# Infinidat/slimfastq

Measured on AMD Instinct MI355X. Metric: MB/s FASTQ compressed, higher is better.
Workload: dtype u8/u32 integer; 1 GPU; synthetic 10M x 150 bp Illumina reads per GPU, full qlts+gens+recs, frozen tables (one chain per lane), -l 3; level=3, block_reads=1024, prior_step=-1, blocks_per_gpu=9766, tables=frozen, chains_per_gpu=253906, raw_bytes_per_gpu=3702038404, parallelism=1 GPU

## Files before the change

### slimfastq_amd/csrc/chains.hip

```cpp
#include "kernels.h"
#include "dev_chain.h"
#include "dev_walk.h"
typedef u32 __attribute__((aligned(1))) u32_any;

#define LAST_QLT 63u
#define QROW_BYTES 256u
#define B2_INIT 0x03030303u

#define QDEC_ROW 72u
__device__ __forceinline__ void qdec_store(u16* row, u32 s, u32 cum) {
    if (s) row[8 + s - 1] = (u16)cum;
    if ((s & 7u) == 0) row[s >> 3] = (u16)cum;
    if (s == 63) row[8 + 63] = 0;
}
__global__ __launch_bounds__(256) void k_qlt_frozen_rows(const u32* __restrict__ rows66, u32 q_rows, u32* __restrict__ qrows, u16* __restrict__ qdec) {
    const u32 lane = threadIdx.x & 63;
    const u32 ctx = blockIdx.x * 4 + (threadIdx.x >> 6);
    if (ctx >= q_rows) return;
    const u32* r = rows66 + (size_t)ctx * 66;
    const u32 slot = r[lane], iend = r[65];
    if (iend == 0) {
        qrows[(size_t)ctx * 64 + lane] = (lane << 10) | (1024u << 16);
        if (qdec) qdec_store(qdec + (size_t)ctx * QDEC_ROW, lane, lane << 10);
        return;
    }
    const u32 sym = slot >> 16, fslot = lane < iend ? (slot & 0xffffu) : 0u;
    const u32 f = (u32)__builtin_amdgcn_ds_permute((int)((lane < iend ? sym : lane) * 4), (int)fslot);
    const u32 x = f + 1;
    u32 S = x;
#pragma unroll
    for (int d = 32; d > 0; d >>= 1) S += (u32)__shfl_xor((int)S, d, 64);
    u32 g = (x << 16) / S;
    g = g ? g : 1u;
    u32 sum = g, best = (g << 6) | (63u - lane);
#pragma unroll
    for (int d = 32; d > 0; d >>= 1) {
        sum += (u32)__shfl_xor((int)sum, d, 64);
        const u32 o = (u32)__shfl_xor((int)best, d, 64); best = o > best ? o : best;
    }
    if (lane == 63u - (best & 63u)) g += 65536u - sum;
    u32 incl = g;
#pragma unroll
    for (int d = 1; d < 64; d <<= 1) { const u32 o = (u32)__shfl_up((int)incl, d, 64); if (lane >= (u32)d) incl += o; }
    qrows[(size_t)ctx * 64 + lane] = (incl - g) | (g << 16);
    if (qdec) qdec_store(qdec + (size_t)ctx * QDEC_ROW, lane, incl - g);
}
void launch_qlt_frozen_rows(const u32* rows66, u32 q_rows, u32* qrows, u16* qdec, hipStream_t st) {
    hipLaunchKernelGGL(k_qlt_frozen_rows, dim3((q_rows + 3) / 4), dim3(256), 0, st, rows66, q_rows, qrows, qdec);
}

#define QH_SYMS 48u
#define QH_ROW_U16 50u
#define QH_MAP_BYTES(q_rows) ((q_rows) / 32u * 8u)
#define QH_EMPTY 0xFFFFFFFFu
__global__ __launch_bounds__(256) void k_hot_totals(const u32* __restrict__ hist, const u32* __restrict__ rows66, u32 q_rows, u32* __restrict__ ctot) {
    const u32 lane = threadIdx.x & 63;
    const u32 ctx = blockIdx.x * 4 + (threadIdx.x >> 6);
    if (ctx >= q_rows) return;
    u32 c = hist[(size_t)ctx * 64 + lane];
#pragma unroll
    for (int d = 32; d > 0; d >>= 1) c += (u32)__shfl_xor((int)c, d, 64);
    const u32 iend = rows66[(size_t)ctx * 66 + 65];
    if (lane == 0) ctot[ctx] = (iend != 0 && iend <= QH_SYMS) ? c : 0u;
}
__global__ __launch_bounds__(1024) void k_hot_select(const u32* __restrict__ ctot, u32 q_rows, u32 want, uint2* __restrict__ map, u32* __restrict__ info) {
    __shared__ u32 red[16];
    __shared__ u32 wbits[2048];
    const u32 t = threadIdx.x, lane = t & 63, wave = t >> 6;
    const u32 nwords = q_rows / 32u;
    u32 c[64];
    u32 mx = 0;
#pragma unroll
    for (u32 k = 0; k < 64; k++) {
        const u32 ctx = k * 1024u + t;
        c[k] = ctx < q_rows ? ctot[ctx] : 0u;
        mx = c[k] > mx ? c[k] : mx;
    }
    auto block_sum = [&](u32 v) {
#pragma unroll
        for (int d = 32; d > 0; d >>= 1) v += (u32)__shfl_xor((int)v, d, 64);
        __syncthreads();
        if (lane == 0) red[wave] = v;
        __syncthreads();
        u32 s2 = 0;
        for (u32 w = 0; w < 16; w++) s2 += red[w];
        return s2;
    };
    auto block_max = [&](u32 v) {
#pragma unroll
        for (int d = 32; d > 0; d >>= 1) { const u32 o = (u32)__shfl_xor((int)v, d, 64); v = o > v ? o : v; }
        __syncthreads();
        if (lane == 0) red[wave] = v;
        __syncthreads();
        u32 s2 = 0;
        for (u32 w = 0; w < 16; w++) s2 = red[w] > s2 ? red[w] : s2;
        return s2;
    };
    u32 lo = 1, hi = block_max(mx) + 1u;
    while (lo < hi) {
        const u32 mid = lo + (hi - lo) / 2u;
        u32 n = 0;
#pragma unroll
        for (u32 k = 0; k < 64; k++) n += c[k] >= mid;
        if (block_sum(n) <= want) hi = mid; else lo = mid + 1u;
    }
    const u32 T = lo;
#pragma unroll
    for (u32 k = 0; k < 64; k++) {
        const u64 m = __ballot(c[k] >= T);
        if (lane == 0) { wbits[k * 32u + wave * 2u] = (u32)m; wbits[k * 32u + wave * 2u + 1u] = (u32)(m >> 32); }
    }
    __syncthreads();
    const u32 b0 = 2u * t < nwords ? wbits[2u * t] : 0u, b1 = 2u * t + 1u < nwords ? wbits[2u * t + 1u] : 0u;
    const u32 mine = (u32)__popc(b0) + (u32)__popc(b1);
    u32 inc = mine;
#pragma unroll
    for (int d = 1; d < 64; d <<= 1) { const u32 o = (u32)__shfl_up((int)inc, d, 64); if (lane >= (u32)d) inc += o; }
    __syncthreads();
    if (lane == 63) red[wave] = inc;
    __syncthreads();
    u32 before = 0, all = 0;
    for (u32 w = 0; w < 16; w++) { const u32 v = red[w]; before += w < wave ? v : 0u; all += v; }
    const u32 rank = before + inc - mine;
    if (t == 0) info[0] = all;
    if (2u * t < nwords) map[2u * t] = make_uint2(b0, rank);
    if (2u * t + 1u < nwords) map[2u * t + 1u] = make_uint2(b1, rank + (u32)__popc(b0));
}
__global__ __launch_bounds__(256) void k_hot_image(const uint2* __restrict__ map, const u32* __restrict__ qrows, u32 q_rows, u16* __restrict__ rows) {
    const u32 lane = threadIdx.x & 63;
    const u32 ctx = blockIdx.x * 4 + (threadIdx.x >> 6);
    if (ctx >= q_rows) return;
    const uint2 mr = map[ctx >> 5];
    const u32 bit = 1u << (ctx & 31u);
    if (!(mr.x & bit)) return;
    const u32 slot = mr.y + (u32)__popc(mr.x & (bit - 1u));
    if (lane < QH_ROW_U16) rows[(size_t)slot * QH_ROW_U16 + lane] = lane <= QH_SYMS ? (u16)FZ_CUM(qrows[(size_t)ctx * 64 + lane]) : (u16)0;
}
void launch_hot_rows(const u32* hist, const u32* rows66, const u32* qrows, u32 q_rows, u32 want, u32* ctot, u8* img, u32* info, hipStream_t st) {
    hipLaunchKernelGGL(k_hot_totals, dim3((q_rows + 3) / 4), dim3(256), 0, st, hist, rows66, q_rows, ctot);
    hipLaunchKernelGGL(k_hot_select, dim3(1), dim3(1024), 0, st, (const u32*)ctot, q_rows, want, reinterpret_cast<uint2*>(img), info);
    hipLaunchKernelGGL(k_hot_image, dim3((q_rows + 3) / 4), dim3(256), 0, st, reinterpret_cast<const uint2*>(img), qrows, q_rows,
                       reinterpret_cast<u16*>(img + QH_MAP_BYTES(q_rows)));
}

#define QHD_ROW_U16 8u
#define QHD_MAX_ROWS 6000u
__global__ __launch_bounds__(256) void k_hot_totals_prior(const u32* __restrict__ rows66, u32 q_rows, u32* __restrict__ ctot) {
    const u32 ctx = blockIdx.x * 256 + threadIdx.x;
    if (ctx >= q_rows) return;
    const u32 iend = rows66[(size_t)ctx * 66 + 65];
    ctot[ctx] = iend != 0 ? rows66[(size_t)ctx * 66 + 64] + 1u : 0u;
}
__global__ __launch_bounds__(256) void k_hot_image_dec(const uint2* __restrict__ map, const u16* __restrict__ qdec, u32 q_rows, u16* __restrict__ rows) {
    const u32 ctx = blockIdx.x * 256 + threadIdx.x;
    if (ctx >= q_rows) return;
// ... 551 lines not shown
        __syncthreads();
    }
}
__device__ __forceinline__ u32 gen_row_of(uint4 n, u32 step) {
    u64 f0 = 3 + (u64)step * n.x, f1 = 3 + (u64)step * n.y, f2 = 3 + (u64)step * n.z, f3 = 3 + (u64)step * n.w;
    while ((f0 | f1 | f2 | f3) > 255) {
        f0 = (f0 >> 1) | (f0 & 1); f1 = (f1 >> 1) | (f1 & 1); f2 = (f2 >> 1) | (f2 & 1); f3 = (f3 >> 1) | (f3 & 1);
    }
    return (u32)f0 | (u32)f1 << 8 | (u32)f2 << 16 | (u32)f3 << 24;
}
__global__ __launch_bounds__(1024) void k_gen_bin_count(const u16* __restrict__ bins, u32* __restrict__ fill, u32 cap, u32 g_bits, u32* __restrict__ cnt,
                                                        u32* __restrict__ rows_out, u32 step) {
    extern __shared__ u32 lds[];
    const u32 sb = gb_slice_bits(g_bits), nctx = 1u << sb, b = blockIdx.x, tid = threadIdx.x;
    u32 n = fill[b]; if (n > cap) n = cap;
    const u16* bin = bins + (size_t)b * cap;
    uint4* slice = reinterpret_cast<uint4*>(cnt + ((size_t)b << (sb + 2)));
    if (!n && !rows_out) return;
    for (u32 at = 0; ; at += 65535u) {
        for (u32 i = tid; i < 2u * nctx; i += 1024u) lds[i] = 0;
        __syncthreads();
        const u32 m = n - at < 65535u ? n - at : 65535u;
        for (u32 i = tid; i < m; i += 1024u) {
            const u32 k = bin[at + i];
            atomicAdd(&lds[k >> 1], 1u << ((k & 1u) * 16u));
        }
        __syncthreads();
        const bool last_chunk = at + m >= n;
        for (u32 i = tid; i < nctx; i += 1024u) {
            const u32 w0 = lds[2 * i], w1 = lds[2 * i + 1];
            if (!(w0 | w1) && !(rows_out && last_chunk)) continue;
            uint4 c = slice[i];
            c.x += w0 & 0xffffu; c.y += w0 >> 16; c.z += w1 & 0xffffu; c.w += w1 >> 16;
            if (w0 | w1) slice[i] = c;
            if (rows_out && last_chunk) rows_out[((size_t)b << sb) + i] = gen_row_of(c, step);
        }
        if (last_chunk) break;
        __syncthreads();
    }
    if (tid == 0) fill[b] = 0;
}
GenBins gen_bins_plan(u32 g_bits, u64 max_keys) {
    GenBins gb; gb.bins = nullptr; gb.fill = nullptr;
    gb.g_bits = g_bits;
    gb.batch = max_keys < GEN_BIN_BATCH ? (max_keys ? max_keys : 1) : GEN_BIN_BATCH;
    const u32 nb = 1u << (g_bits - gb_slice_bits(g_bits));
    gb.cap = (u32)((2ull * ((gb.batch + nb - 1) / nb) + 4096ull + 63ull) & ~63ull);
    gb.bins_bytes = (u64)gb.cap * 2ull * nb; gb.fill_bytes = 4ull * nb;
    return gb;
}
void launch_gen_count_binned(const ChainArgs& a, u32 b0, u32 b1, u64 nrec_range, u32 max_line, const GenBins& gb, u32* cnt, u32* rows_out, u32 step,
                             hipStream_t st, u32 sub) {
    const u32 g_bits = gb.g_bits, sb = gb_slice_bits(g_bits), nb = 1u << (g_bits - sb), cap = gb.cap;
    const u32 dyn2 = (2u << sb) * 4u;
    static u32 allowed = 0;
    if (dyn2 > 65536u && dyn2 > allowed) { (void)hipFuncSetAttribute(reinterpret_cast<const void*>(&k_gen_bin_count), hipFuncAttributeMaxDynamicSharedMemorySize, (int)dyn2); allowed = dyn2; }
    if (nrec_range) {
        u32 stride = gen_count_stride(nrec_range);
        if (sub == 1) { stride *= GEN_PRE; sub = 0; }
        u32 seg_len = 0;
        if (max_line >= 64u) {
            const u64 nsel = (nrec_range + stride - 1) / stride;
            for (u32 sl = 32u; sl < max_line && sl <= 512u; sl *= 2u)
                if (nsel * ((max_line + sl - 1) / sl) <= 524288ull) { seg_len = sl; break; }
        }
        if (!seg_len && max_line > 1024u) seg_len = 512u;
        const u32 segs = seg_len ? (max_line + seg_len - 1) / seg_len : 1u;
        const u64 lanes = ((nrec_range + stride - 1) / stride) * segs;
        const u64 per_lane = seg_len ? seg_len : (max_line ? max_line : 1u);
        u64 lanes_per_batch = gb.batch / per_lane; if (!lanes_per_batch) lanes_per_batch = 1;
        lanes_per_batch = (lanes_per_batch + GB_T - 1) / GB_T * GB_T;
        const u32 dyn1 = (GB_TILE + 2u * nb) * 4u;
        for (u64 id0 = 0; id0 < lanes; id0 += lanes_per_batch) {
            const u64 id1 = id0 + lanes_per_batch < lanes ? id0 + lanes_per_batch : lanes;
            const bool last = id1 >= lanes;
            hipLaunchKernelGGL(k_gen_bin, dim3((u32)((id1 - id0 + GB_T - 1) / GB_T)), dim3(GB_T), dyn1, st, a, b0, b1, stride, seg_len, segs, sub, id0, id1, g_bits, gb.bins, gb.fill, cap, cnt);
            hipLaunchKernelGGL(k_gen_bin_count, dim3(nb), dim3(1024), dyn2, st, (const u16*)gb.bins, gb.fill, cap, g_bits, cnt, last ? rows_out : nullptr, step);
        }
    } else if (rows_out) hipLaunchKernelGGL(k_gen_bin_count, dim3(nb), dim3(1024), dyn2, st, (const u16*)gb.bins, gb.fill, cap, g_bits, cnt, rows_out, step);
}

__global__ __launch_bounds__(256) void k_gen_rows(const u32* __restrict__ cnt, u32* __restrict__ rows, u64 nctx, u32 step) {
    const u64 c = (u64)blockIdx.x * 256 + threadIdx.x;
    if (c >= nctx) return;
    const uint4 n = *reinterpret_cast<const uint4*>(cnt + c * 4);
    u64 f0 = 3 + (u64)step * n.x, f1 = 3 + (u64)step * n.y, f2 = 3 + (u64)step * n.z, f3 = 3 + (u64)step * n.w;
    while ((f0 | f1 | f2 | f3) > 255) {
        f0 = (f0 >> 1) | (f0 & 1); f1 = (f1 >> 1) | (f1 & 1); f2 = (f2 >> 1) | (f2 & 1); f3 = (f3 >> 1) | (f3 & 1);
    }
    rows[c] = (u32)f0 | (u32)f1 << 8 | (u32)f2 << 16 | (u32)f3 << 24;
}
void launch_gen_rows(const u32* cnt, u32* rows, u64 nctx, u32 step, hipStream_t st) {
    hipLaunchKernelGGL(k_gen_rows, dim3((u32)((nctx + 255) / 256)), dim3(256), 0, st, cnt, rows, nctx, step);
}

__device__ __forceinline__ const u32* gen_rows_of(const ChainArgs& a, u32 b) {
    if (!a.g_ngen) return nullptr;
    u32 g = 0;
    while (g + 1 < a.g_ngen && b >= a.g_bound[g + 1]) g++;
    return a.g_rows[g];
}

#define GEN_RING 8
template <int THREADS, bool FLAT>
__global__ __launch_bounds__(THREADS) void k_gen_encode_c(ChainArgs a, u32 c0, u32 c1 ) {
    __shared__ u32 rcp[FLAT ? 1 : 1024];
    __shared__ u8 lut[256];
    __shared__ u32 ring[LaneEncB<THREADS, GEN_RING>::LDS_DWORDS];
    if constexpr (!FLAT) for (u32 i = threadIdx.x; i < 1024; i += THREADS) rcp[i] = i ? rc_recip(i) : 0u;
    for (u32 i = threadIdx.x; i < 256; i += THREADS) lut[i] = (u8)(gen_code_of(i) | (is_lower_base(i) ? 0x20u : 0u));
    __syncthreads();
    const u32 c = c0 + blockIdx.x * THREADS + threadIdx.x;
    const bool live = c < c1;
    ChainPos cp; cp.b = 0; cp.r0 = 0; cp.nrec = 0; cp.sub_lo = cp.sub_len = 0; cp.seg = 0; cp.nseg = 1;
    if (live) { cp = chain_pos(a, c); chain_seg_encode(a, cp); }
    const BlockDesc* d = &a.m.blocks[cp.b];
    LaneEncB<THREADS, GEN_RING> rc; u32 cap = 0;
    u8* outp = live ? chain_region(a, cp, SFQ_S_GEN, 3, 4, cap) : nullptr;
    rc.init(ring, threadIdx.x, outp, cap);
    const u32* rows = (!FLAT && live) ? gen_rows_of(a, cp.b) : nullptr;
    u32 illegal = 0;
    if (a.flat_quads && (FLAT || !__any(rows != nullptr))) {
        illegal = walk_bases_q(a, cp.r0, cp.nrec, live ? d->solid : 0u, lut,
            [&](u32 sym, u32 k) { const u32 bits = 2u * k; rc.encode_bits_if(k ? ~0u : 0u, sym & ((1u << bits) - 1u), 1u, bits); rc.drain(); },
            a.exc_flag, cp.sub_lo, cp.sub_len);
    } else if (FLAT || !__any(rows != nullptr)) {
        const u32 r12 = rc_recip(12u);
        illegal = walk_bases_b(a, cp.r0, cp.nrec, live ? d->solid : 0u, 0u, lut, [&](u32, u32) {},
            [&](u32, u32 code, u32 vm) { rc.encode_if(vm, 3u * code, 3u, 12u, r12); },
            [&]() { rc.drain(); }, a.exc_flag, cp.sub_lo, cp.sub_len);
    } else if constexpr (!FLAT) {
        const u32* rp = rows ? rows : a.g_init;
        const u32 mask = (live && rows) ? (1u << d->gen_bits) - 1u : 0u;
        u32 rv[16];
        illegal = walk_bases_b(a, cp.r0, cp.nrec, live ? d->solid : 0u, mask, lut,
            [&](u32 j, u32 ctx) { rv[j] = rp[ctx]; },
            [&](u32 j, u32 code, u32 vm) {
                const u32 v = rv[j];
                const u32 f0 = v & 0xff, f1 = (v >> 8) & 0xff, f2 = (v >> 16) & 0xff, f3 = v >> 24;
                const u32 tot = (f0 + f1) + (f2 + f3);
                const u32 below = v & ((1u << (8 * code)) - 1u);
                const u32 cum = (below & 0xff) + ((below >> 8) & 0xff) + (below >> 16);
                rc.encode_if(vm, cum, (v >> (8 * code)) & 0xff, tot, rcp[tot]);
            },
            [&]() { rc.drain(); }, a.exc_flag, cp.sub_lo, cp.sub_len);
    }
    if (live) {
        a.csz[c] = rc.finish();
        if (rc.err & 2) atomicMax(&a.m.blocks[cp.b].status, (u32)(-SFQ_E_OVERFLOW));
        else if (rc.err) atomicMax(&a.m.blocks[cp.b].status, (u32)(-SFQ_E_CORRUPT));
        if (illegal) atomicMax(&a.m.blocks[cp.b].status, (u32)(-SFQ_E_GENCHAR));
    }
}
__device__ __forceinline__ uint4 gp_below(u32 n) {
    const u64 lo = n >= 8u ? ~0ull : (1ull << (8u * n)) - 1ull;
    const u64 hi = n >= 16u ? ~0ull : n <= 8u ? 0ull : (1ull << (8u * (n - 8u))) - 1ull;
    return make_uint4((u32)lo, (u32)(lo >> 32), (u32)hi, (u32)(hi >> 32));
}
__device__ __forceinline__ uint4 gp_load16(const u8* buf, u64 nbytes, long long at) {
    if (at >= 0 && (u64)at + 16u <= nbytes) return load16(buf, nbytes, (u64)at);
    u32 w[4] = {0, 0, 0, 0};
    for (u32 i = 0; i < 16; i++) { const long long p = at + (long long)i; if (p >= 0 && (u64)p < nbytes) w[i >> 2] |= (u32)buf[p] << ((i & 3) * 8); }
    return make_uint4(w[0], w[1], w[2], w[3]);
}
__device__ __forceinline__ u32 gp_codes(u32 w, u32 valid, u32& odd, u32& ill) {
    const u32 s1 = w >> 1;
    u32 cd = (s1 ^ (w >> 2)) & 0x03030303u;
    const u32 want = __builtin_amdgcn_perm(0u, 0x47544341u, s1 & 0x03030303u);
    odd = 0; ill = 0;
    if ((want ^ w) & valid) {
        cd = 0;
#pragma unroll
        for (u32 i = 0; i < 4; i++) {
            const u32 ch = (w >> (8u * i)) & 0xffu, g = gen_code_of(ch);
            cd |= (g & 3u) << (8u * i);
            if ((valid >> (8u * i)) & 0xffu) {
                if (g > 3u || is_lower_base(ch)) odd |= 0x80u << (8u * i);
                if (g & 0x10u) ill = 1;
            }
        }
    }
    return cd & valid & 0x03030303u;
}
__device__ __forceinline__ u32 gp_fold(u32 cd) { return cd | (cd >> 6); }
__device__ __forceinline__ u32 gp_nib(u32 t) { return ((t >> 7) * 0x01020408u) >> 24; }
__device__ __forceinline__ u32 gp_bits16(u32 o0, u32 o1, u32 o2, u32 o3) { return gp_nib(o0) | gp_nib(o1) << 4 | gp_nib(o2) << 8 | gp_nib(o3) << 12; }
__global__ __launch_bounds__(256) void k_gen_pack_raw(ChainArgs a, u32 c0, u32 c1) {
    const u32 lane = threadIdx.x & 63u;
    const u32 c = c0 + blockIdx.x * 4u + (threadIdx.x >> 6);
    if (c >= c1) return;
    ChainPos cp = chain_pos(a, c); chain_seg_encode(a, cp);
    const u32 solid = a.m.blocks[cp.b].solid;
    u32 cap = 0;
    u32* out = reinterpret_cast<u32*>(chain_region(a, cp, SFQ_S_GEN, 3, 4, cap));
    const u8* buf = a.st_off ? a.st_buf : a.m.fq;
    const u64 nbytes = a.st_off ? a.st_bytes : a.nbytes;
    u32 done = 0;
    u32 carry = 0;
    u32 illegal = 0;
    for (u32 k0 = 0; k0 < cp.nrec; k0 += 64u) {
        const u32 k = k0 + lane;
        u64 b0 = 0, b1 = 0;
        if (k < cp.nrec) {
            const u64 r = cp.r0 + k;
            if (a.st_off) { b0 = a.st_off[r]; b1 = b0 + a.st_len[r]; }
            else { b0 = a.m.line_off[4 * r + 1] + solid; b1 = a.m.line_off[4 * r + 2] - 1; }
            if (cp.sub_len) {
                if (b1 < b0) b1 = b0;
                const u64 lo = b0 + cp.sub_lo;
                b0 = lo < b1 ? lo : b1;
                b1 = b0 + cp.sub_len < b1 ? b0 + cp.sub_len : b1;
            }
            if (b1 < b0) b1 = b0;
        }
        const u32 len = (u32)(b1 - b0);
        u32 inc = len;
#pragma unroll
        for (int d = 1; d < 64; d <<= 1) { const u32 o = (u32)__shfl_up((int)inc, d, 64); if (lane >= (u32)d) inc += o; }
        const u32 st = inc - len;
        const u32 tot = (u32)__shfl((int)inc, 63, 64);
        const u32 end = done + tot;
        const bool last_chunk = k0 + 64u >= cp.nrec;
        const u32 t0 = done >> 4, t1 = (end + 15u) >> 4;
        for (u32 tb = t0; tb < t1; tb += 64u) {
            const u32 t = tb + lane;
            const u32 d0 = 16u * t;
            const u32 lo = d0 > done ? d0 : done, hi = d0 + 16u < end ? d0 + 16u : end;
            u32 kr = 0;
#pragma unroll
            for (u32 s = 32; s > 0; s >>= 1) { const u32 sk = (u32)__shfl((int)st, (int)(kr + s), 64); if (sk + done <= lo) kr += s; }
            uint4 w = make_uint4(0, 0, 0, 0);
            u32 pos = lo;
            while (__any(pos < hi)) {
                const u32 ks = kr & 63u;
                const u32 sk = (u32)__shfl((int)st, (int)ks, 64) + done, lk = (u32)__shfl((int)len, (int)ks, 64);
                const u64 bk = (u64)__shfl((unsigned long long)b0, (int)ks, 64);
                const u32 e = sk + lk < hi ? sk + lk : hi;
                if (pos < hi && e > pos) {
                    const u32 j = pos - d0;
                    const uint4 v = gp_load16(buf, nbytes, (long long)(bk + (pos - sk)) - (long long)j);
                    const uint4 m0 = gp_below(j), m1 = gp_below(j + (e - pos));
                    w.x = (w.x & ~(m1.x & ~m0.x)) | (v.x & m1.x & ~m0.x);
                    w.y = (w.y & ~(m1.y & ~m0.y)) | (v.y & m1.y & ~m0.y);
                    w.z = (w.z & ~(m1.z & ~m0.z)) | (v.z & m1.z & ~m0.z);
                    w.w = (w.w & ~(m1.w & ~m0.w)) | (v.w & m1.w & ~m0.w);
                    pos = e;
                }
                kr++;
            }
            const bool any = lo < hi;
            const uint4 va = gp_below(any ? hi - d0 : 0u), vb = gp_below(any ? lo - d0 : 0u);
            const uint4 vm = make_uint4(va.x & ~vb.x, va.y & ~vb.y, va.z & ~vb.z, va.w & ~vb.w);
            u32 o0, o1, o2, o3, i0, i1, i2, i3;
            const u32 f0 = gp_fold(gp_codes(w.x, vm.x, o0, i0)), f1 = gp_fold(gp_codes(w.y, vm.y, o1, i1));
            const u32 f2 = gp_fold(gp_codes(w.z, vm.z, o2, i2)), f3 = gp_fold(gp_codes(w.w, vm.w, o3, i3));
            illegal |= i0 | i1 | i2 | i3;
            u32 p01 = __builtin_amdgcn_perm(f1, f0, 0x06020400u), p23 = __builtin_amdgcn_perm(f3, f2, 0x06020400u);
            p01 |= p01 >> 12; p23 |= p23 >> 12;
            u32 code = __builtin_amdgcn_perm(p23, p01, 0x05040100u);
            if (t == t0) code |= carry;
            u32 odd = gp_bits16(o0, o1, o2, o3);
            if (a.exc_flag) {
                while (__any(odd != 0u)) {
                    const u32 jb = odd ? (u32)__builtin_ctz(odd) : 0u;
                    u32 ko = 0;
#pragma unroll
                    for (u32 s = 32; s > 0; s >>= 1) { const u32 sk = (u32)__shfl((int)st, (int)(ko + s), 64); if (sk + done <= d0 + jb) ko += s; }
                    const u32 ke = (u32)__shfl((int)inc, (int)ko, 64) + done;
                    if (odd) {
                        a.exc_flag[cp.r0 + k0 + ko] = 1;
                        odd &= ke - d0 >= 16u ? 0u : ~((1u << (ke - d0)) - 1u);
                    }
                }
            }
            const bool held = t == t1 - 1u && (end & 15u) && !last_chunk;
            if (t < t1 && !held && 4u * t < cap) out[t] = code;
            if (!last_chunk) carry = (end & 15u) ? (u32)__shfl((int)code, (int)((t1 - 1u - tb) & 63u), 64) : 0u;
        }
        done = end;
    }
    if (lane == 0) {
        const u32 n = (done + 3u) >> 2;
        a.csz[c] = n;
        if (n > cap) atomicMax(&a.m.blocks[cp.b].status, (u32)(-SFQ_E_OVERFLOW));
    }
    if (__any(illegal != 0u) && lane == 0) atomicMax(&a.m.blocks[cp.b].status, (u32)(-SFQ_E_GENCHAR));
}
void launch_gen_encode_c(const ChainArgs& a, hipStream_t st, u32 c0, u32 c1, bool flat) {
    constexpr int T = 256;
    if (!c1 || c1 > a.geo.nchains) c1 = a.geo.nchains;
    if (c1 <= c0) return;
    if (a.flat_raw) { hipLaunchKernelGGL(k_gen_pack_raw, dim3((c1 - c0 + 3) / 4), dim3(256), 0, st, a, c0, c1); return; }
    const dim3 grid((c1 - c0 + T - 1) / T);
    if (flat) hipLaunchKernelGGL((k_gen_encode_c<T, true>), grid, dim3(T), 0, st, a, c0, c1);
    else hipLaunchKernelGGL((k_gen_encode_c<T, false>), grid, dim3(T), 0, st, a, c0, c1);
}

__device__ __forceinline__ u32 b2_pick(u32 v, LaneDecQ& rc, const u32* rcp) {
    const u32 f0 = v & 0xff, f1 = (v >> 8) & 0xff, f2 = (v >> 16) & 0xff, f3 = v >> 24;
    const u32 c1 = f0, c2 = f0 + f1, c3 = c2 + f2, tot = c3 + f3;
    u32 r;
    const u32 prob = rc.get_freq(tot, rcp[tot], r);
    const u32 b = (prob >= c1 ? 1u : 0u) + (prob >= c2 ? 1u : 0u) + (prob >= c3 ? 1u : 0u);
    const u32 cum = b == 0 ? 0u : b == 1 ? c1 : b == 2 ? c2 : c3;
    rc.decode(r, cum, (v >> (8 * b)) & 0xff);
    return b;
}
template <int THREADS>
__global__ __launch_bounds__(THREADS) void k_gen_decode_c(ChainArgs a, DecodeArgs da, u32 c0, u32 c1 ) {
    __shared__ u32 rcp[1024];
    for (u32 i = threadIdx.x; i < 1024; i += THREADS) rcp[i] = i ? rc_recip(i) : 0u;
    __syncthreads();
    const u32 c = c0 + blockIdx.x * THREADS + threadIdx.x;
    if (c >= c1) return;
    ChainPos cp = chain_pos(a, c);
    const BlockDesc* d = &a.m.blocks[cp.b];
    LaneDecQ rc; rc.init(da.streams + a.coff[c], a.csz[c], reinterpret_cast<const u8*>(a.qesc));
    const u32* rows = gen_rows_of(a, cp.b);
    const u32 alphabet = d->solid ? 0x33323130u  : 0x54474341u ;
    const u32 mask = (1u << d->gen_bits) - 1u;
    const u32 INIT = 0x007616c7u;
    const u32 r12 = rc_recip(12u);
    u32 n_next = cp.nrec ? da.slen[cp.r0] : 0u; u64 off_next = cp.nrec ? da.soff[cp.r0] : 0ull;
    if (a.seg_len) {
        const u32 ql = da.qlen[cp.r0];
        seg_range(cp, ql > n_next ? ql : n_next);
        const u64 lo = cp.sub_lo < n_next ? cp.sub_lo : n_next;
        n_next = (u32)(n_next - lo < cp.sub_len ? n_next - lo : cp.sub_len); off_next += lo;
    }
    const u8* const raw = da.streams + a.coff[c]; const u32 raw_n = a.csz[c];
    u32 racc = 0, rnb = 0, rat = 0, rbad = 0;
    for (u32 k = 0; k < cp.nrec; k++) {
        const u32 llen = n_next; const u64 off = off_next;
        if (k + 1 < cp.nrec) { n_next = da.slen[cp.r0 + k + 1]; off_next = da.soff[cp.r0 + k + 1]; }
        LaneOut32 out; out.begin(da.seq_stage + off);
        u32 last = INIT;
        if (a.flat_raw) {
            for (u32 i = 0; i < llen; i++) {
                if (rnb == 0) {
                    if (rat + 4u <= raw_n) { racc = *reinterpret_cast<const u32_any*>(raw + rat); rat += 4u; rnb = 32u; }
                    else if (rat < raw_n) { racc = raw[rat++]; rnb = 8u; }
                    else { rbad = 1; racc = 0; rnb = 32u; }
                }
                out.put((alphabet >> (8u * (racc & 3u))) & 0xffu);
                racc >>= 2; rnb -= 2u;
            }
        } else
        if (rows) {
            u32 v = rows[last & mask];
            for (u32 i = 0; i < llen; i++) {
                const uint4 cand = *reinterpret_cast<const uint4*>(rows + ((last << 2) & mask));
                rc.top_up();
                const u32 b = b2_pick(v, rc, rcp);
                out.put((alphabet >> (8 * b)) & 0xff);
                last = (last << 2) | b;
                v = b == 0 ? cand.x : b == 1 ? cand.y : b == 2 ? cand.z : cand.w;
            }
        } else if (a.flat_quads) {
            for (u32 i = 0; i < llen; i += 4u) {
                const u32 k = llen - i < 4u ? llen - i : 4u;
                rc.top_up();
                u32 r;
                const u32 S = rc.get_freq_bits(2u * k, r);
                rc.decode1(r, S, 1u);
                for (u32 j = 0; j < k; j++) out.put((alphabet >> (8u * ((S >> (2u * j)) & 3u))) & 0xffu);
            }
        } else {
            for (u32 i = 0; i < llen; i++) {
                rc.top_up();
                u32 r;
                const u32 prob = rc.get_freq(12u, r12, r);
                const u32 b = (prob >= 3u ? 1u : 0u) + (prob >= 6u ? 1u : 0u) + (prob >= 9u ? 1u : 0u);
                rc.decode1(r, 3u * b, 3u);
                out.put((alphabet >> (8 * b)) & 0xff);
            }
        }
        out.end();
    }
    if (a.flat_raw) { if (rbad || rat != raw_n || (rnb >= 8u) || racc) atomicMax(&a.m.blocks[cp.b].status, (u32)(-SFQ_E_CORRUPT)); }
    else
    if (rc.err) atomicMax(&a.m.blocks[cp.b].status, (u32)(-SFQ_E_CORRUPT));
}
void launch_gen_decode_c(const ChainArgs& a, const DecodeArgs& da, u32 c0, u32 c1, hipStream_t st) {
    constexpr int T = 256;
    if (c1 > a.geo.nchains) c1 = a.geo.nchains;
    if (c1 <= c0) return;
    hipLaunchKernelGGL(k_gen_decode_c<T>, dim3((c1 - c0 + T - 1) / T), dim3(T), 0, st, a, da, c0, c1);
}

#include "dev_rec_lane.h"
#include "dev_wave.h"

struct RecChainPos { u32 b; u64 r0; u32 nrec; };
__device__ __forceinline__ RecChainPos rec_chain_pos(const ChainArgs& a, u32 c) {
    RecChainPos p;
    p.b = c / a.rgeo.cpb;
    const u32 j = c - p.b * a.rgeo.cpb;
    const BlockDesc* d = &a.m.blocks[p.b];
    const u32 k0 = j * a.rgeo.chain_reads;
    p.nrec = k0 < d->nrec ? (d->nrec - k0 < a.rgeo.chain_reads ? d->nrec - k0 : a.rgeo.chain_reads) : 0u;
    p.r0 = d->rec0 + k0;
    return p;
}
__device__ __forceinline__ u8* rec_chain_region(const ChainArgs& a, const RecChainPos& p, u32& cap) {
    const BlockDesc* d = &a.m.blocks[p.b];
    const u64 t0 = a.m.line_off[4 * d->rec0], tc = a.m.line_off[4 * p.r0], te = a.m.line_off[4 * (p.r0 + p.nrec)];
    const u64 lo = ((tc - t0) * 3 / 2 + 3) & ~3ull, hi = ((te - t0) * 3 / 2) & ~3ull;
    cap = hi > lo ? (u32)(hi - lo) : 0u;
    return a.m.arena + d->out_off[SFQ_S_REC] + lo;
}

#define REC_HBUF 128u
#define REC_LDS_ROWS 8u
struct RecFrozenEnc {
    static constexpr bool inband = true;
    const u32* rows; LaneEnc rc;
    u8* lbuf;
    const u16* lmap; const u32* lrows;
    __device__ __forceinline__ void record(u32) {}
    __device__ __forceinline__ const u8* stage(const u8* g, u32 n, u32 k) {
        if (n + 1 > REC_HBUF) return g;
        u8* dst = lbuf + (k & 1u) * REC_HBUF;
        const u32 nw = (n + 4) / 4;
#pragma unroll 8
        for (u32 i = 0; i < nw; i++) reinterpret_cast<u32*>(dst)[i] = reinterpret_cast<const u32_any*>(g)[i];
        return dst;
    }
    __device__ __forceinline__ void put(u32 row, u32 sym) {
        const u32 slot = lmap[row];
        const u32 e = slot != 0xFFFFu ? lrows[slot * 256 + sym] : rows[(size_t)row * 256 + sym];
        rc.encode16(FZ_CUM(e), FZ_FREQ(e));
    }
// ... 1139 lines not shown
```

Measured before the change: 331,200 MB/s.

## Rewrite raw gen packer with per-wave LDS tile and record-parallel loads

The raw genome packing kernel now assigns lanes to records or 16-byte pieces of records and loads each record aligned to its own start. Codes are OR-ed atomically into a per-wave shared-memory tile holding a 4 KB window, which is then flushed to global memory. This replaces the per-output-word binary search and the loop that stitched records together through shuffles. A fast ACGT check skips the per-byte decode unless bad characters appear or the slow path is forced. The cost is LDS atomics, extra wave barriers and more complex windowing logic, with carry handling for records that overflow the window.

```diff
diff --git a/slimfastq_amd/csrc/chains.hip b/slimfastq_amd/csrc/chains.hip
--- a/slimfastq_amd/csrc/chains.hip
+++ b/slimfastq_amd/csrc/chains.hip
@@ -1,6 +1,7 @@
 #include "kernels.h"
 #include "dev_chain.h"
 #include "dev_walk.h"
+#include "dev_wave.h"
 typedef u32 __attribute__((aligned(1))) u32_any;
 
 #define LAST_QLT 63u
@@ -858,42 +859,53 @@
         if (illegal) atomicMax(&a.m.blocks[cp.b].status, (u32)(-SFQ_E_GENCHAR));
     }
 }
+#define GP_WIN 4096u
+#define GP_TILE (GP_WIN / 16u + 1u)
 __device__ __forceinline__ uint4 gp_below(u32 n) {
     const u64 lo = n >= 8u ? ~0ull : (1ull << (8u * n)) - 1ull;
     const u64 hi = n >= 16u ? ~0ull : n <= 8u ? 0ull : (1ull << (8u * (n - 8u))) - 1ull;
     return make_uint4((u32)lo, (u32)(lo >> 32), (u32)hi, (u32)(hi >> 32));
 }
-__device__ __forceinline__ uint4 gp_load16(const u8* buf, u64 nbytes, long long at) {
-    if (at >= 0 && (u64)at + 16u <= nbytes) return load16(buf, nbytes, (u64)at);
-    u32 w[4] = {0, 0, 0, 0};
-    for (u32 i = 0; i < 16; i++) { const long long p = at + (long long)i; if (p >= 0 && (u64)p < nbytes) w[i >> 2] |= (u32)buf[p] << ((i & 3) * 8); }
-    return make_uint4(w[0], w[1], w[2], w[3]);
-}
-__device__ __forceinline__ u32 gp_codes(u32 w, u32 valid, u32& odd, u32& ill) {
+__device__ __forceinline__ void gp_phase() {
+    __builtin_amdgcn_fence(__ATOMIC_RELEASE, "wavefront");
+    __builtin_amdgcn_wave_barrier();
+    __builtin_amdgcn_fence(__ATOMIC_ACQUIRE, "wavefront");
+}
+__device__ __forceinline__ u32 gp_codes(u32 w, u32& bad) {
     const u32 s1 = w >> 1;
-    u32 cd = (s1 ^ (w >> 2)) & 0x03030303u;
-    const u32 want = __builtin_amdgcn_perm(0u, 0x47544341u, s1 & 0x03030303u);
-    odd = 0; ill = 0;
-    if ((want ^ w) & valid) {
-        cd = 0;
-#pragma unroll
-        for (u32 i = 0; i < 4; i++) {
-            const u32 ch = (w >> (8u * i)) & 0xffu, g = gen_code_of(ch);
-            cd |= (g & 3u) << (8u * i);
-            if ((valid >> (8u * i)) & 0xffu) {
-                if (g > 3u || is_lower_base(ch)) odd |= 0x80u << (8u * i);
-                if (g & 0x10u) ill = 1;
-            }
-        }
-    }
-    return cd & valid & 0x03030303u;
-}
-__device__ __forceinline__ u32 gp_fold(u32 cd) { return cd | (cd >> 6); }
-__device__ __forceinline__ u32 gp_nib(u32 t) { return ((t >> 7) * 0x01020408u) >> 24; }
-__device__ __forceinline__ u32 gp_bits16(u32 o0, u32 o1, u32 o2, u32 o3) { return gp_nib(o0) | gp_nib(o1) << 4 | gp_nib(o2) << 8 | gp_nib(o3) << 12; }
+    const u32 want = __builtin_amdgcn_perm(0x4e000000u, 0x47544341u, s1 & 0x07070707u);
+    bad |= (want ^ w) & 0xdfdfdfdfu;
+    return (s1 ^ (w >> 2)) & 0x03030303u;
+}
+__device__ __forceinline__ u32 gp_codes_slow(u32 w, u32& odd, u32& ill) {
+    u32 cd = 0;
+#pragma unroll
+    for (u32 i = 0; i < 4; i++) {
+        const u32 ch = (w >> (8u * i)) & 0xffu, g = gen_code_of(ch);
+        cd |= (g & 3u) << (8u * i);
+        if (g > 3u || is_lower_base(ch)) odd = 1;
+        if (g & 0x10u) ill = 1;
+    }
+    return cd;
+}
+__device__ __forceinline__ u32 gp_pack8(u32 c0, u32 c1) {
+    return __builtin_amdgcn_perm(c1, c0, 0x06040200u) | __builtin_amdgcn_perm(c1, c0, 0x07050301u) << 2;
+}
+__device__ __forceinline__ u32 gp_pack16(u32 c0, u32 c1, u32 c2, u32 c3) {
+    const u32 n0 = gp_pack8(c0, c1), n1 = gp_pack8(c2, c3);
+    return __builtin_amdgcn_perm(n1, n0, 0x06040200u) | __builtin_amdgcn_perm(n1, n0, 0x07050301u) << 4;
+}
 __global__ __launch_bounds__(256) void k_gen_pack_raw(ChainArgs a, u32 c0, u32 c1) {
-    const u32 lane = threadIdx.x & 63u;
-    const u32 c = c0 + blockIdx.x * 4u + (threadIdx.x >> 6);
+    __shared__ u32 tile_s[4][GP_TILE];
+    __shared__ uint4 tab_s[4][64];
+    __shared__ uint4 below_s[17];
+    const u32 lane = threadIdx.x & 63u, wv = threadIdx.x >> 6;
+    u32* tile = tile_s[wv];
+    uint4* tab = tab_s[wv];
+    if (threadIdx.x < 17u) below_s[threadIdx.x] = gp_below(threadIdx.x);
+    for (u32 i = lane; i < GP_TILE; i += 64u) tile[i] = 0;
+    __syncthreads();
+    const u32 c = c0 + blockIdx.x * 4u + wv;
     if (c >= c1) return;
     ChainPos cp = chain_pos(a, c); chain_seg_encode(a, cp);
     const u32 solid = a.m.blocks[cp.b].solid;
@@ -901,11 +913,12 @@
     u32* out = reinterpret_cast<u32*>(chain_region(a, cp, SFQ_S_GEN, 3, 4, cap));
     const u8* buf = a.st_off ? a.st_buf : a.m.fq;
     const u64 nbytes = a.st_off ? a.st_bytes : a.nbytes;
+    const bool slow = rfl(solid) || a.exc_flag;
     u32 done = 0;
-    u32 carry = 0;
+    u32 k0 = 0, roff = 0;
     u32 illegal = 0;
-    for (u32 k0 = 0; k0 < cp.nrec; k0 += 64u) {
-        const u32 k = k0 + lane;
+    while (k0 < cp.nrec) {
+        const u32 kc = k0, k = kc + lane;
         u64 b0 = 0, b1 = 0;
         if (k < cp.nrec) {
             const u64 r = cp.r0 + k;
@@ -918,72 +931,69 @@
                 b1 = b0 + cp.sub_len < b1 ? b0 + cp.sub_len : b1;
             }
             if (b1 < b0) b1 = b0;
-        }
-        const u32 len = (u32)(b1 - b0);
-        u32 inc = len;
-#pragma unroll
-        for (int d = 1; d < 64; d <<= 1) { const u32 o = (u32)__shfl_up((int)inc, d, 64); if (lane >= (u32)d) inc += o; }
-        const u32 st = inc - len;
-        const u32 tot = (u32)__shfl((int)inc, 63, 64);
-        const u32 end = done + tot;
-        const bool last_chunk = k0 + 64u >= cp.nrec;
-        const u32 t0 = done >> 4, t1 = (end + 15u) >> 4;
-        for (u32 tb = t0; tb < t1; tb += 64u) {
-            const u32 t = tb + lane;
-            const u32 d0 = 16u * t;
-            const u32 lo = d0 > done ? d0 : done, hi = d0 + 16u < end ? d0 + 16u : end;
-            u32 kr = 0;
-#pragma unroll
-            for (u32 s = 32; s > 0; s >>= 1) { const u32 sk = (u32)__shfl((int)st, (int)(kr + s), 64); if (sk + done <= lo) kr += s; }
-            uint4 w = make_uint4(0, 0, 0, 0);
-            u32 pos = lo;
-            while (__any(pos < hi)) {
-                const u32 ks = kr & 63u;
-                const u32 sk = (u32)__shfl((int)st, (int)ks, 64) + done, lk = (u32)__shfl((int)len, (int)ks, 64);
-                const u64 bk = (u64)__shfl((unsigned long long)b0, (int)ks, 64);
-                const u32 e = sk + lk < hi ? sk + lk : hi;
-                if (pos < hi && e > pos) {
-                    const u32 j = pos - d0;
-                    const uint4 v = gp_load16(buf, nbytes, (long long)(bk + (pos - sk)) - (long long)j);
-                    const uint4 m0 = gp_below(j), m1 = gp_below(j + (e - pos));
-                    w.x = (w.x & ~(m1.x & ~m0.x)) | (v.x & m1.x & ~m0.x);
-                    w.y = (w.y & ~(m1.y & ~m0.y)) | (v.y & m1.y & ~m0.y);
-                    w.z = (w.z & ~(m1.z & ~m0.z)) | (v.z & m1.z & ~m0.z);
-                    w.w = (w.w & ~(m1.w & ~m0.w)) | (v.w & m1.w & ~m0.w);
-                    pos = e;
+            if (lane == 0) b0 += roff;
+        }
+        const u64 len = b1 - b0;
+        const u32 p0 = done & 15u, room = GP_WIN - p0;
+        const u32 lenc = len < room ? (u32)len : room;
+        const u32 inc = wave_incl_scan(lenc);
+        const u32 st = inc - lenc;
+        const bool part = k < cp.nrec && st < room;
+        const u32 take = part ? (lenc < room - st ? lenc : room - st) : 0u;
+        const u32 n = (u32)__popcll(__ballot(part));
+        const u32 tot = rl(inc, 63) < room ? rl(inc, 63) : room;
+        const bool cut = __ballot(part && len > take) != 0;
+        if (part) tab[lane] = make_uint4((u32)b0, (u32)(b0 >> 32), p0 + st, take);
+        const u32 st_last = rl(st, n - 1u);
+        roff = cut ? (n == 1u ? roff : 0u) + (tot - st_last) : 0u;
+        k0 += cut ? n - 1u : n;
+        const u32 pmax = (rl(wave_incl_scan_max(take), 63) + 15u) >> 4;
+        const u32 P = pmax < 1u ? 1u : pmax > 64u ? 64u : pmax;
+        const u32 rounds = pmax > 64u ? (pmax + 63u) >> 6 : 1u;
+        const float rp = __builtin_amdgcn_rcpf((float)P);
+        const u32 G = (u32)(64.5f * rp), q = (u32)(((float)lane + 0.5f) * rp), jl = lane - q * P;
+        gp_phase();
+        for (u32 g = 0; g < n; g += G) {
+            const u32 r = g + q;
+            const bool on = q < G && r < n;
+            const uint4 e = tab[on ? r : 0u];
+            for (u32 i = 0; i < rounds; i++) {
+                const u32 at = 16u * (jl + i * P);
+                const bool act = on && at < e.w;
+                const u32 nb = act ? (e.w - at < 16u ? e.w - at : 16u) : 0u;
+                uint4 w = make_uint4(0, 0, 0, 0);
+                if (act) w = load16(buf, nbytes, ((u64)e.y << 32 | e.x) + at);
+                const uint4 m = below_s[nb];
+                w.x = ((w.x ^ 0x41414141u) & m.x) ^ 0x41414141u; w.y = ((w.y ^ 0x41414141u) & m.y) ^ 0x41414141u;
+                w.z = ((w.z ^ 0x41414141u) & m.z) ^ 0x41414141u; w.w = ((w.w ^ 0x41414141u) & m.w) ^ 0x41414141u;
+                asm volatile("" : "+v"(w.x), "+v"(w.y), "+v"(w.z), "+v"(w.w));
+                u32 bad = 0;
+                u32 d0 = gp_codes(w.x, bad), d1 = gp_codes(w.y, bad), d2 = gp_codes(w.z, bad), d3 = gp_codes(w.w, bad);
+                if (slow || __any(bad != 0u)) {
+                    u32 odd = 0;
+                    d0 = gp_codes_slow(w.x, odd, illegal); d1 = gp_codes_slow(w.y, odd, illegal);
+                    d2 = gp_codes_slow(w.z, odd, illegal); d3 = gp_codes_slow(w.w, odd, illegal);
+                    if (a.exc_flag && odd) a.exc_flag[cp.r0 + kc + r] = 1;
                 }
-                kr++;
-            }
-            const bool any = lo < hi;
-            const uint4 va = gp_below(any ? hi - d0 : 0u), vb = gp_below(any ? lo - d0 : 0u);
-            const uint4 vm = make_uint4(va.x & ~vb.x, va.y & ~vb.y, va.z & ~vb.z, va.w & ~vb.w);
-            u32 o0, o1, o2, o3, i0, i1, i2, i3;
-            const u32 f0 = gp_fold(gp_codes(w.x, vm.x, o0, i0)), f1 = gp_fold(gp_codes(w.y, vm.y, o1, i1));
-            const u32 f2 = gp_fold(gp_codes(w.z, vm.z, o2, i2)), f3 = gp_fold(gp_codes(w.w, vm.w, o3, i3));
-            illegal |= i0 | i1 | i2 | i3;
-            u32 p01 = __builtin_amdgcn_perm(f1, f0, 0x06020400u), p23 = __builtin_amdgcn_perm(f3, f2, 0x06020400u);
-            p01 |= p01 >> 12; p23 |= p23 >> 12;
-            u32 code = __builtin_amdgcn_perm(p23, p01, 0x05040100u);
-            if (t == t0) code |= carry;
-            u32 odd = gp_bits16(o0, o1, o2, o3);
-            if (a.exc_flag) {
-                while (__any(odd != 0u)) {
-                    const u32 jb = odd ? (u32)__builtin_ctz(odd) : 0u;
-                    u32 ko = 0;
-#pragma unroll
-                    for (u32 s = 32; s > 0; s >>= 1) { const u32 sk = (u32)__shfl((int)st, (int)(ko + s), 64); if (sk + done <= d0 + jb) ko += s; }
-                    const u32 ke = (u32)__shfl((int)inc, (int)ko, 64) + done;
-                    if (odd) {
-                        a.exc_flag[cp.r0 + k0 + ko] = 1;
-                        odd &= ke - d0 >= 16u ? 0u : ~((1u << (ke - d0)) - 1u);
-                    }
+                const u32 code = gp_pack16(d0, d1, d2, d3);
+                if (act) {
+                    const u32 p = e.z + at, s = 2u * (p & 15u);
+                    atomicOr(&tile[p >> 4], code << s);
+                    if (s) atomicOr(&tile[(p >> 4) + 1u], code >> (32u - s));
                 }
             }
-            const bool held = t == t1 - 1u && (end & 15u) && !last_chunk;
-            if (t < t1 && !held && 4u * t < cap) out[t] = code;
-            if (!last_chunk) carry = (end & 15u) ? (u32)__shfl((int)code, (int)((t1 - 1u - tb) & 63u), 64) : 0u;
-        }
-        done = end;
+        }
+        gp_phase();
+        const bool last_chunk = k0 >= cp.nrec;
+        const u32 t0 = done >> 4, nd = last_chunk ? (p0 + tot + 15u) >> 4 : (p0 + tot) >> 4;
+        for (u32 i = lane; i < nd; i += 64u) {
+            const u32 v = atomicExch(&tile[i], 0u);
+            if (4u * (t0 + i) < cap) out[t0 + i] = v;
+        }
+        gp_phase();
+        if (lane == 0 && nd && !last_chunk) tile[0] = atomicExch(&tile[nd], 0u);
+        gp_phase();
+        done += tot;
     }
     if (lane == 0) {
         const u32 n = (done + 3u) >> 2;
```

Result: no change. 337,100 MB/s (median of 4 runs) (+1.8%).
